# prismformore/Multi-Task-Transformer

Measured on NVIDIA H100. Metric: images/sec, higher is better.
Workload: dtype bf16x3 (split-bf16 operands, fp32 accumulate)

## Files before the change

multi-task-transformer_b200/csrc/attention5_tc.cu:

```cuda
#include <math.h>

#include "host_common.h"
#include "ptx.cuh"

namespace mtt {

constexpr int kA5Consumers = 256;
constexpr int kA5Threads = kA5Consumers + 32;
constexpr uint32_t kA5QTile = 128 * 64 * 2;
constexpr uint32_t kA5KVTile = 64 * 64 * 2;
constexpr int kA5Stages = 2;

struct Attn5Params {
  int B, N, H, T;
  float scale_log2;
  __nv_bfloat16* out_hi;
  __nv_bfloat16* out_lo;
  float* prompt_logits;
};

template <int NSPLIT>
__global__ void __launch_bounds__(kA5Threads, 2)
attention5_kernel(const __grid_constant__ CUtensorMap tmq_hi, const __grid_constant__ CUtensorMap tmq_lo,
                  const __grid_constant__ CUtensorMap tmk_hi, const __grid_constant__ CUtensorMap tmk_lo,
                  const Attn5Params p) {
  extern __shared__ uint8_t smem_raw[];
  uint8_t* smem = reinterpret_cast<uint8_t*>((reinterpret_cast<uintptr_t>(smem_raw) + 1023) &
                                             ~static_cast<uintptr_t>(1023));
  uint8_t* sQ = smem;
  uint8_t* sK = sQ + NSPLIT * kA5QTile;
  uint8_t* sV = sK + kA5Stages * NSPLIT * kA5KVTile;
  uint64_t* bars = reinterpret_cast<uint64_t*>(sV + kA5Stages * NSPLIT * kA5KVTile);
  uint64_t* q_full = bars;
  uint64_t* k_full = bars + 1;
  uint64_t* k_empty = k_full + kA5Stages;
  uint64_t* v_full = k_empty + kA5Stages;
  uint64_t* v_empty = v_full + kA5Stages;

  const int tid = threadIdx.x;
  const int warp = tid >> 5;
  const int lane = tid & 31;
  const int C = p.H * 64;
  const int nq = (p.N + 127) / 128;
  const int nkv = (p.N + 63) / 64;
  const int item = blockIdx.x;
  const int qt = item % nq;
  const int h = (item / nq) % p.H;
  const int b = item / (nq * p.H);

  if (tid == kA5Consumers) {
    tma_prefetch_desc(&tmq_hi);
    tma_prefetch_desc(&tmk_hi);
    if (NSPLIT == 2) {
      tma_prefetch_desc(&tmq_lo);
      tma_prefetch_desc(&tmk_lo);
    }
    mbar_init(q_full, 1);
    for (int s = 0; s < kA5Stages; ++s) {
      mbar_init(&k_full[s], 1);
      mbar_init(&k_empty[s], kA5Consumers / 32);
      mbar_init(&v_full[s], 1);
      mbar_init(&v_empty[s], kA5Consumers / 32);
    }
    fence_barrier_init();
  }
  __syncthreads();

  if (warp == kA5Consumers / 32) {
    if (elect_one()) {
      mbar_arrive_expect_tx(q_full, NSPLIT * kA5QTile);
      tma_load_3d(sQ, &tmq_hi, q_full, h * 64, qt * 128, b);
      if (NSPLIT == 2) tma_load_3d(sQ + kA5QTile, &tmq_lo, q_full, h * 64, qt * 128, b);
    }
    __syncwarp();
    for (int j = 0; j < nkv; ++j) {
      const int s = j % kA5Stages;
      const uint32_t ph = (j / kA5Stages) & 1;
      mbar_wait(&k_empty[s], ph ^ 1);
      if (elect_one()) {
        uint8_t* dk = sK + s * NSPLIT * kA5KVTile;
        mbar_arrive_expect_tx(&k_full[s], NSPLIT * kA5KVTile);
        tma_load_3d(dk, &tmk_hi, &k_full[s], C + h * 64, j * 64, b);
        if (NSPLIT == 2) tma_load_3d(dk + kA5KVTile, &tmk_lo, &k_full[s], C + h * 64, j * 64, b);
      }
      __syncwarp();
      mbar_wait(&v_empty[s], ph ^ 1);
      if (elect_one()) {
        uint8_t* dv = sV + s * NSPLIT * kA5KVTile;
        mbar_arrive_expect_tx(&v_full[s], NSPLIT * kA5KVTile);
        tma_load_3d(dv, &tmk_hi, &v_full[s], 2 * C + h * 64, j * 64, b);
        if (NSPLIT == 2) tma_load_3d(dv + kA5KVTile, &tmk_lo, &v_full[s], 2 * C + h * 64, j * 64, b);
      }
      __syncwarp();
    }
    return;
  }

  const int cw = warp >> 2;
  const int rloc = cw * 64 + (warp & 3) * 16 + (lane >> 2);
  const int col0 = 2 * (lane & 3);
  const uint32_t q_hi = smem_u32(sQ) + (uint32_t)cw * 64 * 128;
  const uint32_t q_lo = q_hi + kA5QTile;
  const float sl2 = p.scale_log2;

  float o[32];
#pragma unroll
  for (int i = 0; i < 32; ++i) o[i] = 0.f;
  float m_run[2] = {-INFINITY, -INFINITY};
  float l_run[2] = {0.f, 0.f};

  mbar_wait(q_full, 0);
  for (int j = 0; j < nkv; ++j) {
    const int s = j % kA5Stages;
    const uint32_t ph = (j / kA5Stages) & 1;
    const int kn = min(64, p.N - j * 64);

    float sc[32];
#pragma unroll
    for (int i = 0; i < 32; ++i) sc[i] = 0.f;
    mbar_wait(&k_full[s], ph);
    const uint32_t k_hi = smem_u32(sK + s * NSPLIT * kA5KVTile), k_lo = k_hi + kA5KVTile;
    wgmma_fence_regs(sc);
    wgmma_fence();
#pragma unroll
    for (int ks = 0; ks < 4; ++ks) {
      const uint64_t qdh = gmma_desc_sw128(q_hi + ks * 32), kdh = gmma_desc_sw128(k_hi + ks * 32);
      wgmma_ss_n64<0>(sc, qdh, kdh, 1);
      if (NSPLIT == 2) {
        wgmma_ss_n64<0>(sc, qdh, gmma_desc_sw128(k_lo + ks * 32), 1);
        wgmma_ss_n64<0>(sc, gmma_desc_sw128(q_lo + ks * 32), kdh, 1);
      }
    }
    wgmma_commit();
    wgmma_wait<0>();
    wgmma_fence_regs(sc);
    __syncwarp();
    if (lane == 0) mbar_arrive(&k_empty[s]);

    if (p.prompt_logits) {
#pragma unroll
      for (int hh = 0; hh < 2; ++hh) {
        const int q_row = qt * 128 + rloc + 8 * hh;
        if (q_row < p.T) {
          float* ex = p.prompt_logits + (((long long)b * p.H + h) * p.T + q_row) * p.N + j * 64;
#pragma unroll
          for (int i = 0; i < 8; ++i) {
            const int c = 8 * i + col0;
            if (c < kn) ex[c] = sc[4 * i + 2 * hh];
            if (c + 1 < kn) ex[c + 1] = sc[4 * i + 2 * hh + 1];
          }
        }
      }
    }

    float alpha[2];
#pragma unroll
    for (int hh = 0; hh < 2; ++hh) {
      float mx = -INFINITY;
#pragma unroll
      for (int i = 0; i < 8; ++i) {
#pragma unroll
        for (int e = 0; e < 2; ++e) {
          if (8 * i + col0 + e >= kn) sc[4 * i + 2 * hh + e] = -INFINITY;
          mx = fmaxf(mx, sc[4 * i + 2 * hh + e]);
        }
      }
      mx = fmaxf(mx, __shfl_xor_sync(0xffffffffu, mx, 1));
      mx = fmaxf(mx, __shfl_xor_sync(0xffffffffu, mx, 2));
      const float m_new = fmaxf(m_run[hh], mx * sl2);
      alpha[hh] = ex2_approx(m_run[hh] - m_new);
      m_run[hh] = m_new;
      float sum = 0.f;
#pragma unroll
      for (int i = 0; i < 8; ++i) {
#pragma unroll
        for (int e = 0; e < 2; ++e) {
          const float pv = ex2_approx(fmaf(sc[4 * i + 2 * hh + e], sl2, -m_new));
          sc[4 * i + 2 * hh + e] = pv;
          sum += pv;
        }
      }
      l_run[hh] = l_run[hh] * alpha[hh] + sum;
    }

    uint32_t ph_[4][4], pl_[4][4];
#pragma unroll
    for (int kk = 0; kk < 4; ++kk) {
#pragma unroll
      for (int r = 0; r < 4; ++r) {
        const int i = 2 * kk + (r >> 1), hh = r & 1;
        if (NSPLIT == 2) split_pack2(sc[4 * i + 2 * hh], sc[4 * i + 2 * hh + 1], ph_[kk][r], pl_[kk][r]);
        else ph_[kk][r] = pack_bf16x2(sc[4 * i + 2 * hh], sc[4 * i + 2 * hh + 1]);
      }
    }
    mbar_wait(&v_full[s], ph);
    const uint32_t v_hi = smem_u32(sV + s * NSPLIT * kA5KVTile), v_lo = v_hi + kA5KVTile;
    float pvb[32];
#pragma unroll
    for (int i = 0; i < 32; ++i) pvb[i] = 0.f;
    wgmma_fence_regs(pvb);
    wgmma_fence();
#pragma unroll
    for (int kk = 0; kk < 4; ++kk) {
      if (kk * 16 >= kn) break;
      const uint64_t vdh = gmma_desc_sw128(v_hi + kk * 2048);
      wgmma_rs_n64<1>(pvb, ph_[kk], vdh, kk > 0 ? 1 : 0);
      if (NSPLIT == 2) {
        wgmma_rs_n64<1>(pvb, ph_[kk], gmma_desc_sw128(v_lo + kk * 2048), 1);
        wgmma_rs_n64<1>(pvb, pl_[kk], vdh, 1);
      }
    }
    wgmma_commit();
    wgmma_wait<0>();
    wgmma_fence_regs(pvb);
#pragma unroll
    for (int i = 0; i < 8; ++i)
#pragma unroll
      for (int r = 0; r < 4; ++r) o[4 * i + r] = fmaf(o[4 * i + r], alpha[r >> 1], pvb[4 * i + r]);
    __syncwarp();
    if (lane == 0) mbar_arrive(&v_empty[s]);
  }

#pragma unroll
  for (int hh = 0; hh < 2; ++hh) {
    float l = l_run[hh];
    l += __shfl_xor_sync(0xffffffffu, l, 1);
    l += __shfl_xor_sync(0xffffffffu, l, 2);
    const float inv = 1.0f / l;
    const int q_row = qt * 128 + rloc + 8 * hh;
    if (q_row >= p.N) continue;
    const long long off = ((long long)b * p.N + q_row) * C + h * 64 + col0;
#pragma unroll
    for (int i = 0; i < 8; ++i) {
      uint32_t hv, lv;
      split_pack2(o[4 * i + 2 * hh] * inv, o[4 * i + 2 * hh + 1] * inv, hv, lv);
      *reinterpret_cast<uint32_t*>(p.out_hi + off + 8 * i) = hv;
      if (NSPLIT == 2 || p.out_lo) *reinterpret_cast<uint32_t*>(p.out_lo + off + 8 * i) = lv;
    }
  }
}

template <int NSPLIT>
static int launch_attn5(const CUtensorMap* maps, const Attn5Params& p, cudaStream_t stream) {
  constexpr uint32_t smem = NSPLIT * kA5QTile + 2 * kA5Stages * NSPLIT * kA5KVTile + 1024 + 256;
  static bool attr_set[kMaxDevices] = {};
  const int dev_ = current_device();
  if (!attr_set[dev_]) {
    cudaError_t e = cudaFuncSetAttribute(attention5_kernel<NSPLIT>, cudaFuncAttributeMaxDynamicSharedMemorySize, smem);
    if (e != cudaSuccess)
      return set_error(MTT_ERR_LAUNCH, "attention: cudaFuncSetAttribute: %s", cudaGetErrorString(e));
    attr_set[dev_] = true;
  }
  const int total = ((p.N + 127) / 128) * p.H * p.B;
  attention5_kernel<NSPLIT><<<total, kA5Threads, smem, stream>>>(maps[0], maps[1], maps[2], maps[3], p);
  return check_launch("mtt_attention");
}

int launch_attention5(const mtt_attn_desc* d, cudaStream_t stream) {
  const int C = d->H * 64;
  CUtensorMap maps[4];
  const uint64_t dims[3] = {(uint64_t)3 * C, (uint64_t)d->N, (uint64_t)d->B};
  const uint64_t str[2] = {(uint64_t)3 * C * 2, (uint64_t)d->N * 3 * C * 2};
  const uint32_t qbox[3] = {64, 128, 1};
  const uint32_t kbox[3] = {64, 64, 1};
  int rc;
  if ((rc = make_tmap_bf16(&maps[0], d->qkv_hi, 3, dims, str, qbox))) return rc;
  if ((rc = make_tmap_bf16(&maps[2], d->qkv_hi, 3, dims, str, kbox))) return rc;
  if (d->nsplit == 2) {
    if ((rc = make_tmap_bf16(&maps[1], d->qkv_lo, 3, dims, str, qbox))) return rc;
    if ((rc = make_tmap_bf16(&maps[3], d->qkv_lo, 3, dims, str, kbox))) return rc;
  } else {
    maps[1] = maps[0];
    maps[3] = maps[2];
  }
  Attn5Params p;
  p.B = d->B;
  p.N = d->N;
  p.H = d->H;
  p.T = d->prompt_logits ? d->T : 0;
  p.scale_log2 = d->scale * 1.4426950408889634f;
  p.out_hi = static_cast<__nv_bfloat16*>(d->out_hi);
  p.out_lo = static_cast<__nv_bfloat16*>(d->out_lo);
  p.prompt_logits = d->prompt_logits;
  return d->nsplit == 2 ? launch_attn5<2>(maps, p, stream) : launch_attn5<1>(maps, p, stream);
}

}
```

Measured before the change: 113.2.

## Make attention kernel persistent with ping-pong warpgroups and overlapped S/PV GEMMs

Turns the attention kernel into a persistent kernel with one CTA per SM. Items are scheduled so that partial last query tiles come at the end, and Q is reloaded per item through a q_empty barrier. It adds a 128-thread producer warpgroup with register reallocation (setmaxnreg), deepens the K/V pipeline to 4 stages, and loads Q into registers via ldmatrix so the S GEMM uses the register-operand form. The two consumer warpgroups alternate tensor-core issue through named barriers, and within each the next S GEMM is overlapped with the current PV GEMM and softmax. The aim is to hide softmax and launch/tail costs, at the price of lower occupancy and more complex synchronisation.

```diff
diff --git a/multi-task-transformer_b200/csrc/attention5_tc.cu b/multi-task-transformer_b200/csrc/attention5_tc.cu
--- a/multi-task-transformer_b200/csrc/attention5_tc.cu
+++ b/multi-task-transformer_b200/csrc/attention5_tc.cu
@@ -6,10 +6,11 @@
 namespace mtt {
 
 constexpr int kA5Consumers = 256;
-constexpr int kA5Threads = kA5Consumers + 32;
+constexpr int kA5Threads = kA5Consumers + 128;
 constexpr uint32_t kA5QTile = 128 * 64 * 2;
 constexpr uint32_t kA5KVTile = 64 * 64 * 2;
-constexpr int kA5Stages = 2;
+constexpr int kA5Stages = 4;
+constexpr uint32_t kA5TurnBar = 1;
 
 struct Attn5Params {
   int B, N, H, T;
@@ -19,8 +20,22 @@
   float* prompt_logits;
 };
 
+__device__ __forceinline__ void attn5_item(int item, int nq, int BH, int H, int& qt, int& h, int& b) {
+  const int full = (nq - 1) * BH;
+  int bh;
+  if (item < full) {
+    qt = item % (nq - 1);
+    bh = item / (nq - 1);
+  } else {
+    qt = nq - 1;
+    bh = item - full;
+  }
+  h = bh % H;
+  b = bh / H;
+}
+
 template <int NSPLIT>
-__global__ void __launch_bounds__(kA5Threads, 2)
+__global__ void __launch_bounds__(kA5Threads, 1)
 attention5_kernel(const __grid_constant__ CUtensorMap tmq_hi, const __grid_constant__ CUtensorMap tmq_lo,
                   const __grid_constant__ CUtensorMap tmk_hi, const __grid_constant__ CUtensorMap tmk_lo,
                   const Attn5Params p) {
@@ -32,7 +47,8 @@
   uint8_t* sV = sK + kA5Stages * NSPLIT * kA5KVTile;
   uint64_t* bars = reinterpret_cast<uint64_t*>(sV + kA5Stages * NSPLIT * kA5KVTile);
   uint64_t* q_full = bars;
-  uint64_t* k_full = bars + 1;
+  uint64_t* q_empty = bars + 1;
+  uint64_t* k_full = bars + 2;
   uint64_t* k_empty = k_full + kA5Stages;
   uint64_t* v_full = k_empty + kA5Stages;
   uint64_t* v_empty = v_full + kA5Stages;
@@ -43,12 +59,10 @@
   const int C = p.H * 64;
   const int nq = (p.N + 127) / 128;
   const int nkv = (p.N + 63) / 64;
-  const int item = blockIdx.x;
-  const int qt = item % nq;
-  const int h = (item / nq) % p.H;
-  const int b = item / (nq * p.H);
-
-  if (tid == kA5Consumers) {
+  const int BH = p.B * p.H;
+  const int total = nq * BH;
+
+  if (tid == 0) {
     tma_prefetch_desc(&tmq_hi);
     tma_prefetch_desc(&tmk_hi);
     if (NSPLIT == 2) {
@@ -56,6 +70,7 @@
       tma_prefetch_desc(&tmk_lo);
     }
     mbar_init(q_full, 1);
+    mbar_init(q_empty, kA5Consumers / 32);
     for (int s = 0; s < kA5Stages; ++s) {
       mbar_init(&k_full[s], 1);
       mbar_init(&k_empty[s], kA5Consumers / 32);
@@ -66,178 +81,284 @@
   }
   __syncthreads();
 
-  if (warp == kA5Consumers / 32) {
-    if (elect_one()) {
-      mbar_arrive_expect_tx(q_full, NSPLIT * kA5QTile);
-      tma_load_3d(sQ, &tmq_hi, q_full, h * 64, qt * 128, b);
-      if (NSPLIT == 2) tma_load_3d(sQ + kA5QTile, &tmq_lo, q_full, h * 64, qt * 128, b);
-    }
-    __syncwarp();
-    for (int j = 0; j < nkv; ++j) {
-      const int s = j % kA5Stages;
-      const uint32_t ph = (j / kA5Stages) & 1;
-      mbar_wait(&k_empty[s], ph ^ 1);
+  if (warp < 4) {
+    setmaxnreg_dec<40>();
+    if (warp != 0) return;
+    int s = 0;
+    uint32_t ph = 0;
+    uint32_t qph = 0;
+    for (int item = blockIdx.x; item < total; item += gridDim.x) {
+      int qt, h, b;
+      attn5_item(item, nq, BH, p.H, qt, h, b);
+      mbar_wait(q_empty, qph ^ 1);
       if (elect_one()) {
-        uint8_t* dk = sK + s * NSPLIT * kA5KVTile;
-        mbar_arrive_expect_tx(&k_full[s], NSPLIT * kA5KVTile);
-        tma_load_3d(dk, &tmk_hi, &k_full[s], C + h * 64, j * 64, b);
-        if (NSPLIT == 2) tma_load_3d(dk + kA5KVTile, &tmk_lo, &k_full[s], C + h * 64, j * 64, b);
+        mbar_arrive_expect_tx(q_full, NSPLIT * kA5QTile);
+        tma_load_3d(sQ, &tmq_hi, q_full, h * 64, qt * 128, b);
+        if (NSPLIT == 2) tma_load_3d(sQ + kA5QTile, &tmq_lo, q_full, h * 64, qt * 128, b);
       }
       __syncwarp();
-      mbar_wait(&v_empty[s], ph ^ 1);
-      if (elect_one()) {
-        uint8_t* dv = sV + s * NSPLIT * kA5KVTile;
-        mbar_arrive_expect_tx(&v_full[s], NSPLIT * kA5KVTile);
-        tma_load_3d(dv, &tmk_hi, &v_full[s], 2 * C + h * 64, j * 64, b);
-        if (NSPLIT == 2) tma_load_3d(dv + kA5KVTile, &tmk_lo, &v_full[s], 2 * C + h * 64, j * 64, b);
-      }
-      __syncwarp();
+      qph ^= 1;
+      for (int j = 0; j < nkv; ++j) {
+        mbar_wait(&k_empty[s], ph ^ 1);
+        if (elect_one()) {
+          uint8_t* dk = sK + s * NSPLIT * kA5KVTile;
+          mbar_arrive_expect_tx(&k_full[s], NSPLIT * kA5KVTile);
+          tma_load_3d(dk, &tmk_hi, &k_full[s], C + h * 64, j * 64, b);
+          if (NSPLIT == 2) tma_load_3d(dk + kA5KVTile, &tmk_lo, &k_full[s], C + h * 64, j * 64, b);
+        }
+        __syncwarp();
+        mbar_wait(&v_empty[s], ph ^ 1);
+        if (elect_one()) {
+          uint8_t* dv = sV + s * NSPLIT * kA5KVTile;
+          mbar_arrive_expect_tx(&v_full[s], NSPLIT * kA5KVTile);
+          tma_load_3d(dv, &tmk_hi, &v_full[s], 2 * C + h * 64, j * 64, b);
+          if (NSPLIT == 2) tma_load_3d(dv + kA5KVTile, &tmk_lo, &v_full[s], 2 * C + h * 64, j * 64, b);
+        }
+        __syncwarp();
+        if (++s == kA5Stages) {
+          s = 0;
+          ph ^= 1;
+        }
+      }
     }
     return;
   }
 
-  const int cw = warp >> 2;
+  setmaxnreg_inc<232>();
+  const int cw = (warp - 4) >> 2;
   const int rloc = cw * 64 + (warp & 3) * 16 + (lane >> 2);
   const int col0 = 2 * (lane & 3);
-  const uint32_t q_hi = smem_u32(sQ) + (uint32_t)cw * 64 * 128;
-  const uint32_t q_lo = q_hi + kA5QTile;
+  const uint32_t q_frag = smem_u32(sQ) + (uint32_t)(cw * 64 + (warp & 3) * 16 + (lane & 7) + ((lane >> 3) & 1) * 8) * 128;
+  const int q_chunk = lane >> 4, q_xor = lane & 7;
   const float sl2 = p.scale_log2;
 
-  float o[32];
-#pragma unroll
-  for (int i = 0; i < 32; ++i) o[i] = 0.f;
-  float m_run[2] = {-INFINITY, -INFINITY};
-  float l_run[2] = {0.f, 0.f};
-
-  mbar_wait(q_full, 0);
-  for (int j = 0; j < nkv; ++j) {
-    const int s = j % kA5Stages;
-    const uint32_t ph = (j / kA5Stages) & 1;
-    const int kn = min(64, p.N - j * 64);
-
+  int s = 0;
+  uint32_t ph = 0;
+  uint32_t qph = 0;
+  auto advance = [&] {
+    if (++s == kA5Stages) {
+      s = 0;
+      ph ^= 1;
+    }
+  };
+  auto wait_turn = [&] {
+    if (cw == 0) bar_sync<kA5TurnBar, 256>(); else bar_sync<kA5TurnBar + 1, 256>();
+  };
+  auto pass_turn = [&] {
+    if (cw == 0) bar_arrive<kA5TurnBar + 1, 256>(); else bar_arrive<kA5TurnBar, 256>();
+  };
+  if (cw == 1) pass_turn();
+
+  for (int item = blockIdx.x; item < total; item += gridDim.x) {
+    int qt, h, b;
+    attn5_item(item, nq, BH, p.H, qt, h, b);
+    const bool active = qt * 128 + cw * 64 < p.N;
+
+    uint32_t qf[4][NSPLIT][4];
+    mbar_wait(q_full, qph);
+    qph ^= 1;
+    if (active) {
+#pragma unroll
+      for (int ks = 0; ks < 4; ++ks) {
+        const uint32_t sw = (uint32_t)(((2 * ks + q_chunk) ^ q_xor) << 4);
+#pragma unroll
+        for (int pl = 0; pl < NSPLIT; ++pl) ldmatrix_x4(qf[ks][pl], q_frag + pl * kA5QTile + sw);
+      }
+    }
+    __syncwarp();
+    if (lane == 0) mbar_arrive(q_empty);
+
+    if (!active) {
+      wait_turn();
+      pass_turn();
+      for (int j = 0; j < nkv; ++j) {
+        wait_turn();
+        pass_turn();
+        mbar_wait(&k_full[s], ph);
+        __syncwarp();
+        if (lane == 0) mbar_arrive(&k_empty[s]);
+        mbar_wait(&v_full[s], ph);
+        __syncwarp();
+        if (lane == 0) mbar_arrive(&v_empty[s]);
+        advance();
+      }
+      continue;
+    }
+
+    float o[32];
+#pragma unroll
+    for (int i = 0; i < 32; ++i) o[i] = 0.f;
+    float m_run[2] = {-INFINITY, -INFINITY};
+    float l_run[2] = {0.f, 0.f};
     float sc[32];
-#pragma unroll
-    for (int i = 0; i < 32; ++i) sc[i] = 0.f;
-    mbar_wait(&k_full[s], ph);
-    const uint32_t k_hi = smem_u32(sK + s * NSPLIT * kA5KVTile), k_lo = k_hi + kA5KVTile;
-    wgmma_fence_regs(sc);
-    wgmma_fence();
-#pragma unroll
-    for (int ks = 0; ks < 4; ++ks) {
-      const uint64_t qdh = gmma_desc_sw128(q_hi + ks * 32), kdh = gmma_desc_sw128(k_hi + ks * 32);
-      wgmma_ss_n64<0>(sc, qdh, kdh, 1);
-      if (NSPLIT == 2) {
-        wgmma_ss_n64<0>(sc, qdh, gmma_desc_sw128(k_lo + ks * 32), 1);
-        wgmma_ss_n64<0>(sc, gmma_desc_sw128(q_lo + ks * 32), kdh, 1);
-      }
-    }
-    wgmma_commit();
+    float alpha[2];
+
+    auto issue_s = [&] {
+#pragma unroll
+      for (int i = 0; i < 32; ++i) sc[i] = 0.f;
+      mbar_wait(&k_full[s], ph);
+      const uint32_t k_hi = smem_u32(sK + s * NSPLIT * kA5KVTile), k_lo = k_hi + kA5KVTile;
+      wgmma_fence_regs(sc);
+      wgmma_fence();
+#pragma unroll
+      for (int ks = 0; ks < 4; ++ks) {
+        const uint64_t kdh = gmma_desc_sw128(k_hi + ks * 32);
+        wgmma_rs_n64<0>(sc, qf[ks][0], kdh, 1);
+        if (NSPLIT == 2) {
+          wgmma_rs_n64<0>(sc, qf[ks][0], gmma_desc_sw128(k_lo + ks * 32), 1);
+          wgmma_rs_n64<0>(sc, qf[ks][NSPLIT - 1], kdh, 1);
+        }
+      }
+      wgmma_commit();
+    };
+    auto softmax = [&](int j, float (&a)[2]) {
+      wgmma_fence_regs(sc);
+      __syncwarp();
+      if (lane == 0) mbar_arrive(&k_empty[s]);
+      const int kn = min(64, p.N - j * 64);
+      if (p.prompt_logits) {
+#pragma unroll
+        for (int hh = 0; hh < 2; ++hh) {
+          const int q_row = qt * 128 + rloc + 8 * hh;
+          if (q_row < p.T) {
+            float* ex = p.prompt_logits + (((long long)b * p.H + h) * p.T + q_row) * p.N + j * 64;
+#pragma unroll
+            for (int i = 0; i < 8; ++i) {
+              const int c = 8 * i + col0;
+              if (c < kn) ex[c] = sc[4 * i + 2 * hh];
+              if (c + 1 < kn) ex[c + 1] = sc[4 * i + 2 * hh + 1];
+            }
+          }
+        }
+      }
+#pragma unroll
+      for (int hh = 0; hh < 2; ++hh) {
+        float mx = -INFINITY;
+#pragma unroll
+        for (int i = 0; i < 8; ++i) {
+#pragma unroll
+          for (int e = 0; e < 2; ++e) {
+            if (8 * i + col0 + e >= kn) sc[4 * i + 2 * hh + e] = -INFINITY;
+            mx = fmaxf(mx, sc[4 * i + 2 * hh + e]);
+          }
+        }
+        mx = fmaxf(mx, __shfl_xor_sync(0xffffffffu, mx, 1));
+        mx = fmaxf(mx, __shfl_xor_sync(0xffffffffu, mx, 2));
+        const float m_new = fmaxf(m_run[hh], mx * sl2);
+        a[hh] = ex2_approx(m_run[hh] - m_new);
+        m_run[hh] = m_new;
+        float sum = 0.f;
+#pragma unroll
+        for (int i = 0; i < 8; ++i) {
+#pragma unroll
+          for (int e = 0; e < 2; ++e) {
+            const float pv = ex2_approx(fmaf(sc[4 * i + 2 * hh + e], sl2, -m_new));
+            sc[4 * i + 2 * hh + e] = pv;
+            sum += pv;
+          }
+        }
+        l_run[hh] = l_run[hh] * a[hh] + sum;
+      }
+    };
+
+    uint32_t pf[4][NSPLIT][4];
+    auto pack_p = [&] {
+#pragma unroll
+      for (int kk = 0; kk < 4; ++kk) {
+#pragma unroll
+        for (int r = 0; r < 4; ++r) {
+          const int i = 2 * kk + (r >> 1), hh = r & 1;
+          if (NSPLIT == 2) split_pack2(sc[4 * i + 2 * hh], sc[4 * i + 2 * hh + 1], pf[kk][0][r], pf[kk][NSPLIT - 1][r]);
+          else pf[kk][0][r] = pack_bf16x2(sc[4 * i + 2 * hh], sc[4 * i + 2 * hh + 1]);
+        }
+      }
+    };
+
+    float pvb[32];
+    auto issue_pv = [&](int sv, uint32_t phv) {
+      mbar_wait(&v_full[sv], phv);
+      const uint32_t v_hi = smem_u32(sV + sv * NSPLIT * kA5KVTile), v_lo = v_hi + kA5KVTile;
+#pragma unroll
+      for (int i = 0; i < 32; ++i) pvb[i] = 0.f;
+      wgmma_fence_regs(pvb);
+      wgmma_fence();
+#pragma unroll
+      for (int kk = 0; kk < 4; ++kk) {
+        const uint64_t vdh = gmma_desc_sw128(v_hi + kk * 2048);
+        wgmma_rs_n64<1>(pvb, pf[kk][0], vdh, kk > 0 ? 1 : 0);
+        if (NSPLIT == 2) {
+          wgmma_rs_n64<1>(pvb, pf[kk][0], gmma_desc_sw128(v_lo + kk * 2048), 1);
+          wgmma_rs_n64<1>(pvb, pf[kk][NSPLIT - 1], vdh, 1);
+        }
+      }
+      wgmma_commit();
+    };
+    auto fold_pv = [&](int sv) {
+      wgmma_fence_regs(pvb);
+#pragma unroll
+      for (int kk = 0; kk < 4; ++kk)
+#pragma unroll
+        for (int pl = 0; pl < NSPLIT; ++pl) wgmma_fence_regs(pf[kk][pl]);
+      __syncwarp();
+      if (lane == 0) mbar_arrive(&v_empty[sv]);
+#pragma unroll
+      for (int i = 0; i < 8; ++i)
+#pragma unroll
+        for (int r = 0; r < 4; ++r) o[4 * i + r] = fmaf(o[4 * i + r], alpha[r >> 1], pvb[4 * i + r]);
+    };
+
+    wait_turn();
+    issue_s();
+    pass_turn();
     wgmma_wait<0>();
-    wgmma_fence_regs(sc);
-    __syncwarp();
-    if (lane == 0) mbar_arrive(&k_empty[s]);
-
-    if (p.prompt_logits) {
-#pragma unroll
-      for (int hh = 0; hh < 2; ++hh) {
-        const int q_row = qt * 128 + rloc + 8 * hh;
-        if (q_row < p.T) {
-          float* ex = p.prompt_logits + (((long long)b * p.H + h) * p.T + q_row) * p.N + j * 64;
-#pragma unroll
-          for (int i = 0; i < 8; ++i) {
-            const int c = 8 * i + col0;
-            if (c < kn) ex[c] = sc[4 * i + 2 * hh];
-            if (c + 1 < kn) ex[c + 1] = sc[4 * i + 2 * hh + 1];
-          }
-        }
-      }
-    }
-
-    float alpha[2];
+    softmax(0, alpha);
+    pack_p();
+    for (int j = 0; j + 1 < nkv; ++j) {
+      const int sv = s;
+      const uint32_t phv = ph;
+      advance();
+      wait_turn();
+      issue_s();
+      issue_pv(sv, phv);
+      pass_turn();
+      float alpha_next[2];
+      wgmma_wait<1>();
+      softmax(j + 1, alpha_next);
+      wgmma_wait<0>();
+      fold_pv(sv);
+      pack_p();
+      alpha[0] = alpha_next[0];
+      alpha[1] = alpha_next[1];
+    }
+    {
+      const int sv = s;
+      wait_turn();
+      issue_pv(sv, ph);
+      pass_turn();
+      advance();
+      wgmma_wait<0>();
+      fold_pv(sv);
+    }
+
 #pragma unroll
     for (int hh = 0; hh < 2; ++hh) {
-      float mx = -INFINITY;
+      float l = l_run[hh];
+      l += __shfl_xor_sync(0xffffffffu, l, 1);
+      l += __shfl_xor_sync(0xffffffffu, l, 2);
+      const float inv = 1.0f / l;
+      const int q_row = qt * 128 + rloc + 8 * hh;
+      if (q_row >= p.N) continue;
+      const long long off = ((long long)b * p.N + q_row) * C + h * 64 + col0;
 #pragma unroll
       for (int i = 0; i < 8; ++i) {
-#pragma unroll
-        for (int e = 0; e < 2; ++e) {
-          if (8 * i + col0 + e >= kn) sc[4 * i + 2 * hh + e] = -INFINITY;
-          mx = fmaxf(mx, sc[4 * i + 2 * hh + e]);
-        }
-      }
-      mx = fmaxf(mx, __shfl_xor_sync(0xffffffffu, mx, 1));
-      mx = fmaxf(mx, __shfl_xor_sync(0xffffffffu, mx, 2));
-      const float m_new = fmaxf(m_run[hh], mx * sl2);
-      alpha[hh] = ex2_approx(m_run[hh] - m_new);
-      m_run[hh] = m_new;
-      float sum = 0.f;
-#pragma unroll
-      for (int i = 0; i < 8; ++i) {
-#pragma unroll
-        for (int e = 0; e < 2; ++e) {
-          const float pv = ex2_approx(fmaf(sc[4 * i + 2 * hh + e], sl2, -m_new));
-          sc[4 * i + 2 * hh + e] = pv;
-          sum += pv;
-        }
-      }
-      l_run[hh] = l_run[hh] * alpha[hh] + sum;
-    }
-
-    uint32_t ph_[4][4], pl_[4][4];
-#pragma unroll
-    for (int kk = 0; kk < 4; ++kk) {
-#pragma unroll
-      for (int r = 0; r < 4; ++r) {
-        const int i = 2 * kk + (r >> 1), hh = r & 1;
-        if (NSPLIT == 2) split_pack2(sc[4 * i + 2 * hh], sc[4 * i + 2 * hh + 1], ph_[kk][r], pl_[kk][r]);
-        else ph_[kk][r] = pack_bf16x2(sc[4 * i + 2 * hh], sc[4 * i + 2 * hh + 1]);
-      }
-    }
-    mbar_wait(&v_full[s], ph);
-    const uint32_t v_hi = smem_u32(sV + s * NSPLIT * kA5KVTile), v_lo = v_hi + kA5KVTile;
-    float pvb[32];
-#pragma unroll
-    for (int i = 0; i < 32; ++i) pvb[i] = 0.f;
-    wgmma_fence_regs(pvb);
-    wgmma_fence();
-#pragma unroll
-    for (int kk = 0; kk < 4; ++kk) {
-      if (kk * 16 >= kn) break;
-      const uint64_t vdh = gmma_desc_sw128(v_hi + kk * 2048);
-      wgmma_rs_n64<1>(pvb, ph_[kk], vdh, kk > 0 ? 1 : 0);
-      if (NSPLIT == 2) {
-        wgmma_rs_n64<1>(pvb, ph_[kk], gmma_desc_sw128(v_lo + kk * 2048), 1);
-        wgmma_rs_n64<1>(pvb, pl_[kk], vdh, 1);
-      }
-    }
-    wgmma_commit();
-    wgmma_wait<0>();
-    wgmma_fence_regs(pvb);
-#pragma unroll
-    for (int i = 0; i < 8; ++i)
-#pragma unroll
-      for (int r = 0; r < 4; ++r) o[4 * i + r] = fmaf(o[4 * i + r], alpha[r >> 1], pvb[4 * i + r]);
-    __syncwarp();
-    if (lane == 0) mbar_arrive(&v_empty[s]);
-  }
-
-#pragma unroll
-  for (int hh = 0; hh < 2; ++hh) {
-    float l = l_run[hh];
-    l += __shfl_xor_sync(0xffffffffu, l, 1);
-    l += __shfl_xor_sync(0xffffffffu, l, 2);
-    const float inv = 1.0f / l;
-    const int q_row = qt * 128 + rloc + 8 * hh;
-    if (q_row >= p.N) continue;
-    const long long off = ((long long)b * p.N + q_row) * C + h * 64 + col0;
-#pragma unroll
-    for (int i = 0; i < 8; ++i) {
-      uint32_t hv, lv;
-      split_pack2(o[4 * i + 2 * hh] * inv, o[4 * i + 2 * hh + 1] * inv, hv, lv);
-      *reinterpret_cast<uint32_t*>(p.out_hi + off + 8 * i) = hv;
-      if (NSPLIT == 2 || p.out_lo) *reinterpret_cast<uint32_t*>(p.out_lo + off + 8 * i) = lv;
-    }
-  }
+        uint32_t hv, lv;
+        split_pack2(o[4 * i + 2 * hh] * inv, o[4 * i + 2 * hh + 1] * inv, hv, lv);
+        *reinterpret_cast<uint32_t*>(p.out_hi + off + 8 * i) = hv;
+        if (NSPLIT == 2 || p.out_lo) *reinterpret_cast<uint32_t*>(p.out_lo + off + 8 * i) = lv;
+      }
+    }
+  }
+  if (cw == 0) wait_turn();
 }
 
 template <int NSPLIT>
@@ -252,7 +373,8 @@
     attr_set[dev_] = true;
   }
   const int total = ((p.N + 127) / 128) * p.H * p.B;
-  attention5_kernel<NSPLIT><<<total, kA5Threads, smem, stream>>>(maps[0], maps[1], maps[2], maps[3], p);
+  const int grid = total < sm_count() ? total : sm_count();
+  attention5_kernel<NSPLIT><<<grid, kA5Threads, smem, stream>>>(maps[0], maps[1], maps[2], maps[3], p);
   return check_launch("mtt_attention");
 }
 
```

Result: faster. 118.1 (median of 6 runs) (+4.3%).
